# mduhme/fusion-gcn

Hardware: AMD Instinct MI355X
Metric: clips/sec (N,C,T,V,M)=(64,3,300,25,2) fwd+bwd (higher is better)
Workload: dtype f32 (products from exact 3-way bf16 splits; see notes.dtype); 1 GPU; AGCN 10-block fwd+bwd, NTU-RGB-D graph, synthetic (N,C,T,V,M)=(64,3,300,25,2), 60 classes, train-mode BatchNorm, CrossEntropy, all parameter gradients; global_batch=64, per_gpu_batch=64, parallelism=dp1, launch=hipgraph, input_pipeline=one HBM-resident batch, init_override=gcn1.bn.weight=1.0 (reference: 1e-6); see notes

## Files before the change

fusion_gcn_amd/csrc/fgcn_tconv.hip:

```cpp
#include "fgcn_tile.hpp"
#include <type_traits>

namespace fgcn {

struct HaloP {
    const float* in;
    float* out;
    const float* w4;
    const float* bias;
    float* stats;
    long long Mv;
    unsigned in_bytes, w_bytes, out_bytes;
    unsigned w_plane_bytes;
    int tiles_m, tiles_n, per_xcd;
    int Tv, V, K, N, ld_in, ld_out;
    FastDiv dV, dTvV, dTv;
    int T_in_full, in_s, in_o, Th_in;
    int T_out_full, out_s, out_o, Th_out;
    int taps, tb, tc;
    int dmin, halo_rows;
    int accumulate;
    const float* bn_a;
    const unsigned char* bn_mask;
    const float* bn_vec;
    const float* fin_vec;
    const float* fin_res;
    float* fin_out;
    unsigned char* fin_mask;
    const float* ep_vec;
    const float* ep_res;
    const float* ep_rvec;
    unsigned* in_amax;
    int stats_rows;
};

#ifndef FGCN_PROBE_HALO
#define FGCN_PROBE_HALO 0
#endif
#ifndef FGCN_HALO_RING
#define FGCN_HALO_RING 4
#endif
#ifndef FGCN_HALO_PF64
#define FGCN_HALO_PF64 1
#endif
constexpr int HAS = 36;
constexpr int HALO_MAX_STAGE = 13;
constexpr int XSB = 80;
using u32x4 = __attribute__((ext_vector_type(4))) unsigned int;

__device__ __forceinline__ f32x4 buf_load4(__amdgpu_buffer_rsrc_t r, unsigned voff, unsigned soff) {
    return __builtin_bit_cast(f32x4, __builtin_amdgcn_raw_buffer_load_b128(r, voff, soff, 0));
}

template <int NT, int MINB, int MM>
__global__ __launch_bounds__(256, MINB) void conv_halo_kernel(HaloP p) {
    extern __shared__ __attribute__((aligned(16))) float Ah[];
    const int tid = threadIdx.x, lane = tid & 63, wave = tid >> 6;
    const int l31 = lane & 31, h = lane >> 5;
    int bm, bn;
    if (p.per_xcd > 0) {
        const int vid = xcd_tile(blockIdx.x, p.per_xcd);
        if (vid >= p.tiles_m * p.tiles_n) return;
        bm = vid / p.tiles_n;
        bn = vid - bm * p.tiles_n;
    } else {
        bm = blockIdx.x;
        bn = blockIdx.y;
    }
    const long long m0 = (long long)bm * 128;
    const int n0 = bn * 32 * NT;
    const int V = p.V, TvV = p.Tv * p.V;
    const unsigned k4b = (tid & 7) * 16;

    const __amdgpu_buffer_rsrc_t rin = buffer_rsrc(p.in, p.in_bytes);
    const __amdgpu_buffer_rsrc_t rw = buffer_rsrc(p.w4, p.w_bytes);

    const long long mrow = m0 + wave * 32 + l31;
    const bool row_ok = mrow < p.Mv;
    const int th_lane = row_ok ? (int)(((unsigned)mrow / (unsigned)V) % (unsigned)p.Tv) : 0;

    unsigned src_off[HALO_MAX_STAGE];
    const int nstage = (p.halo_rows + 31) >> 5;
#pragma unroll
    for (int i = 0; i < HALO_MAX_STAGE; ++i) {
        src_off[i] = 0x80000000u;
        const int r = (tid >> 3) + 32 * i;
        const long long hv = m0 + (long long)p.dmin * V + r;
        if (i < nstage && hv >= 0 && hv < p.Mv) {
            const unsigned hu = (unsigned)hv;
            const int n = (int)(hu / (unsigned)TvV);
            const int rem = (int)(hu - (unsigned)n * (unsigned)TvV);
            const int th = (int)((unsigned)rem / (unsigned)V);
            const int v = rem - th * V;
            const int fr = th * p.in_s + p.in_o;
            if (th < p.Th_in && fr < p.T_in_full)
                src_off[i] = (unsigned)(((((long long)n * p.T_in_full + fr) * V + v) * p.ld_in) * 4) + k4b;
        }
    }

    f32x16 acc[NT];
#pragma unroll
    for (int i = 0; i < NT; ++i) acc[i] = zero16();

    const int IT = p.taps * 4;
    const int K4 = p.K >> 2;
    const int col = n0 + l31;
    unsigned wvoff[NT];
#pragma unroll
    for (int nt = 0; nt < NT; ++nt) wvoff[nt] = (unsigned)(((long long)h * p.N + col + nt * 32) * 16);
    const float* arow = &Ah[(wave * 32 + l31) * HAS + 4 * h];

    auto w_soff = [&](int it, int kc) -> unsigned {
        const int j = it >> 2, q = it & 3;
        return (unsigned)(((long long)(j * K4 + (kc >> 2) + 2 * q) * p.N) * 16);
    };
    auto a_read = [&](int it, bool& ok) -> f32x4 {
        const int j = it >> 2, q = it & 3;
        const int d = j * p.tb + p.tc;
        const int ts = th_lane + d;
        ok = row_ok && ts >= 0 && ts < p.Th_in;
        return *reinterpret_cast<const f32x4*>(arow + (d - p.dmin) * V * HAS + 8 * q);
    };

    for (int kc = 0; kc < p.K; kc += 32) {
        __syncthreads();
        {
            f32x4 stage[HALO_MAX_STAGE];
#pragma unroll
            for (int i = 0; i < HALO_MAX_STAGE; ++i)
                if (i < nstage) stage[i] = buf_load4(rin, src_off[i], (unsigned)kc * 4);
#pragma unroll
            for (int i = 0; i < HALO_MAX_STAGE; ++i) {
                const int r = (tid >> 3) + 32 * i;
                if (i < nstage && r < p.halo_rows) *reinterpret_cast<f32x4*>(&Ah[r * HAS + (tid & 7) * 4]) = stage[i];
            }
        }
        __syncthreads();

        f32x4 b0[NT], b1[NT];
        {
            const unsigned so = w_soff(0, kc);
#pragma unroll
            for (int nt = 0; nt < NT; ++nt) b0[nt] = buf_load4(rw, wvoff[nt], so);
        }
        bool ok0, ok1;
        f32x4 a0 = a_read(0, ok0), a1;
        for (int it = 0; it < IT; it += 2) {
            {
                const unsigned so = w_soff(it + 1, kc);
#pragma unroll
                for (int nt = 0; nt < NT; ++nt) b1[nt] = buf_load4(rw, wvoff[nt], so);
            }
            a1 = a_read(it + 1, ok1);
            if (!ok0) a0 = f32x4{0.f, 0.f, 0.f, 0.f};
            if constexpr (MM != 0) {
                const Frag<MM> ap = make_frag<MM>(a0);
#pragma unroll
                for (int nt = 0; nt < NT; ++nt) acc[nt] = mfma_frag<MM>(ap, make_frag<MM>(b0[nt]), acc[nt]);
            } else {
#pragma unroll
                for (int e = 0; e < 4; ++e)
#pragma unroll
                    for (int nt = 0; nt < NT; ++nt) acc[nt] = mfma32(a0[e], b0[nt][e], acc[nt]);
            }
            if (it + 2 < IT) {
                const unsigned so = w_soff(it + 2, kc);
#pragma unroll
                for (int nt = 0; nt < NT; ++nt) b0[nt] = buf_load4(rw, wvoff[nt], so);
                a0 = a_read(it + 2, ok0);
            }
            if (!ok1) a1 = f32x4{0.f, 0.f, 0.f, 0.f};
            if constexpr (MM != 0) {
                const Frag<MM> ap = make_frag<MM>(a1);
#pragma unroll
                for (int nt = 0; nt < NT; ++nt) acc[nt] = mfma_frag<MM>(ap, make_frag<MM>(b1[nt]), acc[nt]);
            } else {
#pragma unroll
                for (int e = 0; e < 4; ++e)
#pragma unroll
                    for (int nt = 0; nt < NT; ++nt) acc[nt] = mfma32(a1[e], b1[nt][e], acc[nt]);
            }
        }
    }


    const bool plain_out = p.out_s == 1 && p.out_o == 0 && p.T_out_full == p.Tv && p.Th_out == p.Tv;
    constexpr unsigned OOB = 0x80000000u;
    const __amdgpu_buffer_rsrc_t rout = buffer_rsrc(p.out, p.out_bytes);
    const __amdgpu_buffer_rsrc_t rbias = buffer_rsrc((p.bias ? p.bias : p.w4), p.bias ? (unsigned)p.N * 4u : 0u);
    float ssum[NT], ssq[NT], bv[NT];
#pragma unroll
    for (int nt = 0; nt < NT; ++nt) {
        ssum[nt] = 0.f;
        ssq[nt] = 0.f;
        bv[nt] = __builtin_bit_cast(float, __builtin_amdgcn_raw_buffer_load_b32(
                                               rbias, col + nt * 32 < p.N ? (unsigned)(col + nt * 32) * 4u : OOB, 0, 0));
    }
    unsigned rowoff[16];
#pragma unroll
    for (int r = 0; r < 16; ++r) {
        const long long m = m0 + wave * 32 + acc_row(r, lane);
        bool ok = m < p.Mv;
        unsigned orow = (unsigned)(ok ? m : 0);
        if (!plain_out) {
            const int n = (int)(orow / (unsigned)TvV);
            const int rem = (int)(orow - (unsigned)n * (unsigned)TvV);
            const int th = (int)((unsigned)rem / (unsigned)V);
            const int v = rem - th * V;
            ok = ok && th < p.Th_out;
            orow = (unsigned)((n * p.T_out_full + th * p.out_s + p.out_o) * V + v);
        }
        rowoff[r] = ok ? orow * (unsigned)p.ld_out * 4u : OOB;
    }
    auto epilogue = [&](auto acc_c) {
        constexpr bool ACC = decltype(acc_c)::value;
#pragma unroll
        for (int nt = 0; nt < NT; ++nt) {
            const int c = col + nt * 32;
            const unsigned coff = c < p.N ? (unsigned)c * 4u : OOB;
            float old[16];
#pragma unroll
            for (int r = 0; r < 16; ++r) {
                old[r] = 0.f;
                if constexpr (ACC)
                    old[r] = __builtin_bit_cast(float, __builtin_amdgcn_raw_buffer_load_b32(
                        rout, (rowoff[r] == OOB || coff == OOB) ? OOB : rowoff[r] + coff, 0, 0));
            }
#pragma unroll
            for (int r = 0; r < 16; ++r) {
                const unsigned off = (rowoff[r] == OOB || coff == OOB) ? OOB : rowoff[r] + coff;
                const float val = acc[nt][r] + bv[nt] + old[r];
                __builtin_amdgcn_raw_buffer_store_b32(__builtin_bit_cast(unsigned, val), rout, off, 0, 0);
                const float kept = off != OOB ? val : 0.f;
                ssum[nt] += kept;
                ssq[nt] += kept * kept;
            }
        }
    };
    if (p.accumulate) epilogue(std::true_type{});
    else epilogue(std::false_type{});
    if (p.stats) {
        constexpr int BN = 32 * NT;
        __syncthreads();
        float* red = Ah;
#pragma unroll
        for (int nt = 0; nt < NT; ++nt) {
            const float a = ssum[nt] + __shfl_xor(ssum[nt], 32);
            const float b = ssq[nt] + __shfl_xor(ssq[nt], 32);
            if (lane < 32) {
                red[(0 * 4 + wave) * BN + nt * 32 + lane] = a;
                red[(1 * 4 + wave) * BN + nt * 32 + lane] = b;
            }
        }
        __syncthreads();
        if (tid < 2 * BN) {
            const int which = tid / BN, c = tid - which * BN;
            if (n0 + c < p.N)
                p.stats[((long long)bm * 2 + which) * p.N + n0 + c] =
                    red[(which * 4 + 0) * BN + c] + red[(which * 4 + 1) * BN + c] + red[(which * 4 + 2) * BN + c] +
                    red[(which * 4 + 3) * BN + c];
        }
    }
}

template <int NT, int KC, int NP, int EPI = 0, bool FIN = false, int WR = 2, bool STR = false, int IN16 = 0>
__global__ __launch_bounds__(256, (NP == 1 && !FIN && EPI != 4) ? 3 : 2) void conv_halo_x3k32_kernel(HaloP p) {
    static_assert(!IN16 || (NP == 1 && !FIN), "bfloat16 input: the one-part kernel without the fused input stage");
    static_assert(IN16 != 2 || EPI == 0, "bfloat16 output: the plain store epilogue");
    constexpr bool O16 = IN16 == 2;
    static_assert(!(STR && EPI == 3), "an accumulating epilogue stores plainly");
    static_assert(WR == 2 || (WR == 4 && KC == 32 && !FIN), "wave arrangement: 2 x 2, or 4 x 1 for the tap form");
    static_assert(!FIN || KC == 32, "the fused input stage is built for the tap form (32-channel chunks)");
    static_assert((EPI == 0 || EPI == 2 || EPI == 3 || EPI == 4) && !(FIN && EPI != 0),
                  "epilogue: store / store + BatchNorm-backward sums / accumulate / inference output stage");
    constexpr int MTW = WR == 4 ? 3 : 4;
    constexpr int BMR = WR * 16 * MTW;
    static_assert(NP == 1 || NP == 2 || NP == 3, "one or three bf16 parts per operand, or two f16 parts (FGCN_PRODUCTS_F16X2)");
    static_assert(!(FIN && NP == 2), "the fused input stage is not built for the f16x2 products");
    static_assert((NT == 1 || NT == 2 || (NT == 4 && WR == 4)) && (KC == 32 || KC == 64), "wave tile is 64 rows x 32 or 64 columns (48 x 128 as 4 x 1 waves)");
    constexpr int XS = KC * 2;
    auto swz = [](int r) -> unsigned { return KC == 32 ? (unsigned)(r & 4) << 3 : (unsigned)(r & 6) << 4; };
    constexpr int TPR = KC / 4;
    constexpr int RPP = 256 / TPR;
    constexpr int SPC = KC / 32;
    constexpr bool PF = KC == 64 || (NT == 1 && NP == 3 && !FIN && FGCN_HALO_PF64);
    constexpr int NST = KC == 64 ? 8 : HALO_MAX_STAGE;
    constexpr int NU = 2 * NT;
#ifndef FGCN_HALO_RING_NP1
#define FGCN_HALO_RING_NP1 4
#endif
    constexpr int RS = (FGCN_HALO_RING == 4 && NU == 4 && (NP >= 2 || FGCN_HALO_RING_NP1 == 4) && (EPI != 2 || WR == 4) && !FIN) ? 4 : 2;
    constexpr unsigned OOB = 0x80000000u;
    extern __shared__ __attribute__((aligned(16))) float Ah[];
    const int tid = threadIdx.x, lane = tid & 63, wave = __builtin_amdgcn_readfirstlane(tid >> 6);
    const int l15 = lane & 15, g4 = lane >> 4;
    const int wr = WR == 4 ? wave : wave >> 1, wc = WR == 4 ? 0 : wave & 1;
    int bm = blockIdx.x, bn = blockIdx.y;
    if (p.per_xcd > 0) {
        const int vid = xcd_tile(blockIdx.x, p.per_xcd);
        if (vid >= p.tiles_m * p.tiles_n) return;
        bm = vid / p.tiles_n;
        bn = vid - bm * p.tiles_n;
    }
    const int m0 = bm * BMR;
    const int Mv = (int)p.Mv;
    constexpr int BN = (4 / WR) * NT * 32;
    const int n0 = bn * BN;
    const int V = p.V, TvV = p.Tv * p.V;
    const unsigned k4b = (tid % TPR) * 16;

    const __amdgpu_buffer_rsrc_t rin = buffer_rsrc(p.in, p.in_bytes);
    const __amdgpu_buffer_rsrc_t rw = buffer_rsrc((reinterpret_cast<const unsigned char*>(p.w4) + (NP == 2 ? 16 : 0)), p.w_bytes);
    constexpr int EA_NONE = 1000;
    const int ew = NP == 2 ? min(scale_exp_for(*reinterpret_cast<const unsigned*>(p.w4)), 126) : 0;
    int ea = EA_NONE, abound = 0;

    bool row_ok[MTW];
    int th_lane[MTW];
#pragma unroll
    for (int mt = 0; mt < MTW; ++mt) {
        const int mrow = m0 + wr * (16 * MTW) + mt * 16 + l15;
        row_ok[mt] = mrow < Mv;
        const unsigned fr_all = fastdiv(row_ok[mt] ? (unsigned)mrow : 0u, p.dV);
        th_lane[mt] = (int)(fr_all - fastdiv(fr_all, p.dTv) * (unsigned)p.Tv);
    }

    unsigned src_off[NST];
    const int nstage = (p.halo_rows + RPP - 1) / RPP;
#pragma unroll
    for (int i = 0; i < NST; ++i) {
        src_off[i] = OOB;
        const int r = tid / TPR + RPP * i;
        const int hv = m0 + p.dmin * V + r;
        if (i < nstage && hv >= 0 && hv < Mv) {
            const unsigned hu = (unsigned)hv;
            const int n = (int)fastdiv(hu, p.dTvV);
            const int rem = (int)(hu - (unsigned)n * (unsigned)TvV);
            const int th = (int)fastdiv((unsigned)rem, p.dV);
            const int v = rem - th * V;
            const int fr = th * p.in_s + p.in_o;
            if (th < p.Th_in && fr < p.T_in_full)
                src_off[i] = (unsigned)(((n * p.T_in_full + fr) * V + v) * p.ld_in) * 4u + k4b;
        }
    }

    f32x4 acc[MTW][NU];
#pragma unroll
    for (int mt = 0; mt < MTW; ++mt)
#pragma unroll
        for (int nu = 0; nu < NU; ++nu) acc[mt][nu] = f32x4{0.f, 0.f, 0.f, 0.f};

    const int col = n0 + wc * NT * 32 + l15;
    unsigned wvoff[NU];
#pragma unroll
    for (int nu = 0; nu < NU; ++nu) wvoff[nu] = (unsigned)(((long long)g4 * p.N + col + nu * 16) * 16);

    unsigned char* Xh = reinterpret_cast<unsigned char*>(Ah);
    const unsigned plane = (unsigned)p.halo_rows * XS;
    const int xrow = wr * (16 * MTW) + l15;
    const int IT2 = p.taps * SPC;
    const int K8 = p.K >> 3;
    bool probe_started = false;
    auto load_w = [&](u32x4v (&dst)[NP], int nu, int it, int kc) {
        if (it >= IT2) {
            it -= IT2;
            kc += KC;
        }
        if (kc >= p.K) {
            it = 0;
            kc = 0;
        }
        const int j = it / SPC, s2 = it - j * SPC;
        const unsigned so = (unsigned)(((long long)(j * K8 + (kc >> 3) + 4 * s2) * p.N) * 16);
        if ((FGCN_PROBE_HALO & 16) && probe_started) return;
#pragma unroll
        for (int pl = 0; pl < NP; ++pl)
            dst[pl] = __builtin_amdgcn_raw_buffer_load_b128(rw, wvoff[nu], so + pl * p.w_plane_bytes, 0);
    };
    auto load_a = [&](u32x4v (&dst)[NP], int mt, int it) {
        if ((FGCN_PROBE_HALO & 8) && it > 0) return;
        const int j = it / SPC, s2 = it - j * SPC;
        const int d = j * p.tb + p.tc;
        const int r = xrow + (d - p.dmin) * V + mt * 16;
        const unsigned char* src = Xh + r * XS + ((unsigned)(16 * g4 + 64 * s2) ^ swz(r));
        const int ts = th_lane[mt] + d;
        const bool ok = row_ok[mt] && ts >= 0 && ts < p.Th_in;
#pragma unroll
        for (int pl = 0; pl < NP; ++pl) {
            const u32x4v v = *reinterpret_cast<const u32x4v*>(src + pl * plane);
            dst[pl] = ok ? v : u32x4v{0u, 0u, 0u, 0u};
        }
    };

    f32x4 stage[NST], stage2[FIN ? NST : 1];
    constexpr int HALF = FIN ? (NST + 1) / 2 : NST;
    auto fetch = [&](int kc, int lo = 0, int hi = 64) {
#pragma unroll
        for (int i = 0; i < NST; ++i)
            if (i >= lo && i < hi && i < nstage) {
                if constexpr (IN16) {
                    const u32x2 h2 = __builtin_bit_cast(u32x2, __builtin_amdgcn_raw_buffer_load_b64(rin, src_off[i] == OOB ? OOB : src_off[i] >> 1, (unsigned)kc * 2, 0));
                    const unsigned b0 = h2[0], b1 = h2[1];
                    stage[i] = f32x4{__builtin_bit_cast(float, b0), __builtin_bit_cast(float, b1), 0.f, 0.f};
                    continue;
                }
                stage[i] = buf_load4(rin, src_off[i], (unsigned)kc * 4);
                if constexpr (FIN)
                    stage2[i] = buf_load4(buffer_rsrc(p.fin_res, p.in_bytes), src_off[i],
                                          (unsigned)kc * 4);
            }
    };
    auto deposit = [&](int kc, int lo = 0, int hi = 64) {
        const float a_scale = (NP == 2 && ea != EA_NONE) ? exp2i(ea) : 1.f;
        f32x4 fsc = {0.f, 0.f, 0.f, 0.f}, fsh = fsc;
        const __amdgpu_buffer_rsrc_t rgo = buffer_rsrc((FIN ? (void*)p.fin_out : (void*)p.out), FIN ? p.in_bytes : 0u);
        const __amdgpu_buffer_rsrc_t rgm = buffer_rsrc((FIN ? (void*)p.fin_mask : (void*)p.out), FIN ? p.in_bytes >> 5 : 0u);
        const int own0 = -p.dmin * V;
        if constexpr (FIN) {
            fsc = *reinterpret_cast<const f32x4*>(p.fin_vec + 2 * p.K + kc + (tid % TPR) * 4);
            fsh = *reinterpret_cast<const f32x4*>(p.fin_vec + 3 * p.K + kc + (tid % TPR) * 4);
        }
#pragma unroll
        for (int i = 0; i < NST; ++i) {
            if (i < lo || i >= hi) continue;
            const int r = tid / TPR + RPP * i;
            if constexpr (FIN) {
                if (i < nstage) {
                    const bool live = src_off[i] != OOB;
                    f32x4 v = stage[i] * fsc + fsh + stage2[i];
#pragma unroll
                    for (int e = 0; e < 4; ++e) v[e] = live ? fmaxf(v[e], 0.f) : 0.f;
                    stage[i] = v;
                    const bool mine = live && bn == 0 && r >= own0 && r < own0 + BMR;
                    __builtin_amdgcn_raw_buffer_store_b128(__builtin_bit_cast(u32x4, v), rgo, mine ? src_off[i] : OOB,
                                                           (unsigned)kc * 4, 0);
                    unsigned w = ((v[0] > 0.f ? 1u : 0u) | (v[1] > 0.f ? 2u : 0u) | (v[2] > 0.f ? 4u : 0u) | (v[3] > 0.f ? 8u : 0u))
                                 << (4 * (lane & 7));
                    w |= (unsigned)__shfl_xor((int)w, 1);
                    w |= (unsigned)__shfl_xor((int)w, 2);
                    w |= (unsigned)__shfl_xor((int)w, 4);
                    __builtin_amdgcn_raw_buffer_store_b32(w, rgm, (mine && (lane & 7) == 0) ? (src_off[i] + (unsigned)kc * 4) >> 5 : OOB,
                                                          0, 0);
                }
            }
            if (i < nstage && r < p.halo_rows) {
                u32x2 ph, pm, pl;
                unsigned char* dst = Xh + r * XS + ((unsigned)((tid % TPR) * 8) ^ swz(r));
                if constexpr (NP == 2) {
                    split2h_x4(stage[i] * a_scale, ph, pm);
                    *reinterpret_cast<u32x2*>(dst) = ph;
                    *reinterpret_cast<u32x2*>(dst + plane) = pm;
                    continue;
                }
                if constexpr (IN16) {
                    const float e0 = stage[i][0], e1 = stage[i][1];
                    *reinterpret_cast<u32x2*>(dst) = u32x2{__builtin_bit_cast(unsigned, e0), __builtin_bit_cast(unsigned, e1)};
                    continue;
                }
                split3_x4(stage[i], ph, pm, pl);
                *reinterpret_cast<u32x2*>(dst) = ph;
                if constexpr (NP == 3) {
                    *reinterpret_cast<u32x2*>(dst + plane) = pm;
                    *reinterpret_cast<u32x2*>(dst + 2 * plane) = pl;
                }
            }
        }
    };

    u32x4v a[MTW][NP], wq[RS][NP];
#pragma unroll
    for (int nu = 0; nu < RS - 1; ++nu) load_w(wq[nu], nu, 0, 0);
    if constexpr (PF) fetch(0);
    float* smax = reinterpret_cast<float*>(Xh + NP * plane);
    auto chunk_max = [&]() {
        float m = 0.f;
#pragma unroll
        for (int i = 0; i < NST; ++i)
            if (i < nstage)
                m = fmaxf(fmaxf(m, fmaxf(fabsf(stage[i][0]), fabsf(stage[i][1]))), fmaxf(fabsf(stage[i][2]), fabsf(stage[i][3])));
#pragma unroll
        for (int d = 32; d >= 1; d >>= 1) m = fmaxf(m, __shfl_xor(m, d));
        if (lane == 0) smax[wave] = m;
    };
    for (int kc = 0; kc < p.K; kc += KC) {
        if constexpr (NP == 2 && PF) chunk_max();
        __syncthreads();
        if constexpr (FIN) {
            fetch(kc, 0, HALF);
            deposit(kc, 0, HALF);
            fetch(kc, HALF, NST);
            deposit(kc, HALF, NST);
        } else if ((FGCN_PROBE_HALO & 4) && probe_started) {
        } else {
            if constexpr (!PF) fetch(kc);
            if constexpr (NP == 2) {
                if constexpr (!PF) {
                    chunk_max();
                    __syncthreads();
                }
                const unsigned mb = __builtin_bit_cast(unsigned, fmaxf(fmaxf(smax[0], smax[1]), fmaxf(smax[2], smax[3])));
                const int ec = __builtin_amdgcn_readfirstlane((mb >> 23) == 0u ? EA_NONE : min(scale_exp_for(mb), 126));
                if (p.in_amax && tid == 0 && bn == 0) atomicMax(p.in_amax, mb);
                if (ec != EA_NONE && ec != ea) {
                    int d = ea == EA_NONE ? 0 : ec - ea;
                    if (d > 120 - abound) d = 120 - abound;
                    if (ea == EA_NONE) ea = ec;
                    else if (d != 0) {
                        const float f = exp2i(d);
#pragma unroll
                        for (int mt = 0; mt < MTW; ++mt)
#pragma unroll
                            for (int nu = 0; nu < NU; ++nu) acc[mt][nu] *= f;
                        ea += d;
                        abound += d;
                    }
                }
                abound = (abound > 44 ? abound : 44) + 1;
            }
            deposit(kc);
        }
        __syncthreads();
        if constexpr (PF) {
            if (kc + KC < p.K) fetch(kc + KC);
        }
#pragma unroll
        for (int mt = 0; mt < MTW; ++mt) load_a(a[mt], mt, 0);
#pragma unroll 1
        for (int it = 0; it < IT2; ++it) {
            const int itn = it + 1 < IT2 ? it + 1 : it;
#pragma unroll
            for (int nu = 0; nu < NU; ++nu) {
                const int t = nu + RS - 1;
                if (t < NU) load_w(wq[t % RS], t, it, kc);
                else load_w(wq[t % RS], t - NU, it + 1, kc);
#pragma unroll
                for (int mt = 0; mt < MTW; ++mt) {
                    if constexpr ((FGCN_PROBE_HALO & 2) != 0) acc[mt][nu][0] += __builtin_bit_cast(float, a[mt][0][0] ^ wq[nu % RS][0][0] ^ a[mt][NP - 1][3] ^ wq[nu % RS][NP - 1][3]);
                    else if constexpr (NP == 3) acc[mt][nu] = mfma_x3_k32(a[mt], wq[nu % RS], acc[mt][nu]);
                    else if constexpr (NP == 2) acc[mt][nu] = mfma_h2_k32(a[mt], wq[nu % RS], acc[mt][nu]);
                    else acc[mt][nu] = mfma_bf16_k32(a[mt][0], wq[nu % RS][0], acc[mt][nu]);
                    if (nu == NU - 1) load_a(a[mt], mt, itn);
                }
            }
        }
        probe_started = true;
    }

    __builtin_amdgcn_sched_barrier(0);
    const bool plain_out = p.out_s == 1 && p.out_o == 0 && p.T_out_full == p.Tv && p.Th_out == p.Tv;
    const __amdgpu_buffer_rsrc_t rout = buffer_rsrc(p.out, p.out_bytes);
    const __amdgpu_buffer_rsrc_t rbias = buffer_rsrc((p.bias ? p.bias : p.w4), p.bias ? (unsigned)p.N * 4u : 0u);
    float ssum[NU], ssq[NU], bv[NU];
    unsigned coff[NU];
    const float un_a = (NP == 2 && ea != EA_NONE) ? exp2i(-ea) : 1.f, un_w = NP == 2 ? exp2i(-ew) : 1.f;
    constexpr bool bnb = EPI == 2;
    const __amdgpu_buffer_rsrc_t rba = buffer_rsrc((bnb ? p.bn_a : p.out), p.out_bytes);
    const __amdgpu_buffer_rsrc_t rbm = buffer_rsrc((bnb ? (const void*)p.bn_mask : (const void*)p.out), p.out_bytes >> 5);
    const __amdgpu_buffer_rsrc_t rbv = buffer_rsrc((bnb ? p.bn_vec : p.w4), bnb ? (unsigned)p.N * 8u : 0u);
    float bmean[NU], brstd[NU];
#pragma unroll
    for (int nu = 0; nu < NU; ++nu) {
        ssum[nu] = 0.f;
        ssq[nu] = 0.f;
        coff[nu] = col + nu * 16 < p.N ? (unsigned)(col + nu * 16) * 4u : OOB;
        bv[nu] = __builtin_bit_cast(float, __builtin_amdgcn_raw_buffer_load_b32(rbias, coff[nu], 0, 0));
        bmean[nu] = bnb ? __builtin_bit_cast(float, __builtin_amdgcn_raw_buffer_load_b32(rbv, coff[nu], 0, 0)) : 0.f;
        brstd[nu] = bnb ? __builtin_bit_cast(float, __builtin_amdgcn_raw_buffer_load_b32(rbv, coff[nu], (unsigned)p.N * 4u, 0)) : 0.f;
    }
    unsigned rowoff[MTW][4];
#pragma unroll
    for (int mt = 0; mt < MTW; ++mt)
#pragma unroll
        for (int r = 0; r < 4; ++r) {
            const int m = m0 + wr * (16 * MTW) + mt * 16 + 4 * g4 + r;
            bool ok = m < Mv;
            unsigned orow = (unsigned)(ok ? m : 0);
            if (!plain_out) {
                const int n = (int)fastdiv(orow, p.dTvV);
                const int rem = (int)(orow - (unsigned)n * (unsigned)TvV);
                const int th = (int)fastdiv((unsigned)rem, p.dV);
                const int v = rem - th * V;
                ok = ok && th < p.Th_out;
                orow = (unsigned)((n * p.T_out_full + th * p.out_s + p.out_o) * V + v);
            }
            rowoff[mt][r] = ok ? orow * (unsigned)p.ld_out * 4u : OOB;
        }
    float av[bnb ? 2 : 1][NU][4];
    unsigned mbits[bnb ? 2 : 1][NU][4];
    auto load_bn = [&](int mt, float (&a_)[NU][4], unsigned (&m_)[NU][4]) {
#pragma unroll
        for (int nu = 0; nu < NU; ++nu)
#pragma unroll
            for (int r = 0; r < 4; ++r) {
                const unsigned off = (rowoff[mt][r] == OOB || coff[nu] == OOB) ? OOB : rowoff[mt][r] + coff[nu];
                a_[nu][r] = __builtin_bit_cast(float, __builtin_amdgcn_raw_buffer_load_b32(rba, off, 0, 0));
                m_[nu][r] = (unsigned)__builtin_amdgcn_raw_buffer_load_b8(rbm, off == OOB ? OOB : off >> 5, 0, 0);
            }
    };
    constexpr bool fep = EPI == 4;
    constexpr bool ldacc = EPI == 3 || fep;
    const __amdgpu_buffer_rsrc_t rold = fep ? buffer_rsrc((p.ep_res ? (const void*)p.ep_res : (const void*)p.out), p.ep_res ? p.out_bytes : 0u)
                                            : rout;
    float esc[NU], esh[NU], rsc[NU], rsh[NU];
    if constexpr (fep) {
        const __amdgpu_buffer_rsrc_t rv = buffer_rsrc(p.ep_vec, (unsigned)p.N * 16u);
        const __amdgpu_buffer_rsrc_t rrv = buffer_rsrc((p.ep_rvec ? p.ep_rvec : p.ep_vec), p.ep_rvec ? (unsigned)p.N * 16u : 0u);
        const float res_unit = p.ep_rvec ? 0.f : 1.f;
#pragma unroll
        for (int nu = 0; nu < NU; ++nu) {
            esc[nu] = __builtin_bit_cast(float, __builtin_amdgcn_raw_buffer_load_b32(rv, coff[nu], (unsigned)p.N * 8u, 0));
            esh[nu] = __builtin_fmaf(bv[nu], esc[nu], __builtin_bit_cast(float, __builtin_amdgcn_raw_buffer_load_b32(rv, coff[nu], (unsigned)p.N * 12u, 0)));
            rsc[nu] = __builtin_bit_cast(float, __builtin_amdgcn_raw_buffer_load_b32(rrv, coff[nu], (unsigned)p.N * 8u, 0)) + res_unit;
            rsh[nu] = __builtin_bit_cast(float, __builtin_amdgcn_raw_buffer_load_b32(rrv, coff[nu], (unsigned)p.N * 12u, 0));
        }
    }
    float oldv[ldacc ? 2 : 1][NU][4];
    auto load_old = [&](int mt, float (&o_)[NU][4]) {
#pragma unroll
        for (int nu = 0; nu < NU; ++nu)
#pragma unroll
            for (int r = 0; r < 4; ++r)
                o_[nu][r] = __builtin_bit_cast(float, __builtin_amdgcn_raw_buffer_load_b32(
                    rold, (rowoff[mt][r] == OOB || coff[nu] == OOB) ? OOB : rowoff[mt][r] + coff[nu], 0, 0));
    };
    if constexpr (bnb) load_bn(0, av[0], mbits[0]);
    if constexpr (ldacc) load_old(0, oldv[0]);
#pragma unroll
    for (int mt = 0; mt < MTW; ++mt) {
        if constexpr (bnb) {
            if (mt + 1 < MTW) load_bn(mt + 1, av[(mt + 1) & 1], mbits[(mt + 1) & 1]);
        }
        if constexpr (ldacc) {
            if (mt + 1 < MTW) load_old(mt + 1, oldv[(mt + 1) & 1]);
        }
        if constexpr (O16) {
            const bool odd = lane & 1;
#pragma unroll
            for (int rp = 0; rp < 4; rp += 2) {
#pragma unroll
                for (int nu = 0; nu < NU; ++nu) {
                    const unsigned off0 = (rowoff[mt][rp] == OOB || coff[nu] == OOB) ? OOB : rowoff[mt][rp] + coff[nu];
                    const unsigned off1 = (rowoff[mt][rp + 1] == OOB || coff[nu] == OOB) ? OOB : rowoff[mt][rp + 1] + coff[nu];
                    const float v0 = acc[mt][nu][rp] + bv[nu], v1 = acc[mt][nu][rp + 1] + bv[nu];
                    const float other = lane_xor1(odd ? v0 : v1);
                    const unsigned pk = odd ? pack_bf16x2(other, v1) : pack_bf16x2(v0, other);
                    const unsigned mine = odd ? off1 : off0;
                    __builtin_amdgcn_raw_buffer_store_b32(pk, rout, mine == OOB ? OOB : (mine - (odd ? 4u : 0u)) >> 1, 0, STR ? FGCN_STORE_AUX : 0);
                    const float k0 = off0 != OOB ? v0 : 0.f, k1 = off1 != OOB ? v1 : 0.f;
                    ssum[nu] += k0;
                    ssq[nu] = __builtin_fmaf(k0, k0, ssq[nu]);
                    ssum[nu] += k1;
                    ssq[nu] = __builtin_fmaf(k1, k1, ssq[nu]);
                }
            }
            continue;
        }
#pragma unroll
        for (int r = 0; r < 4; ++r) {
#pragma unroll
            for (int nu = 0; nu < NU; ++nu) {
                const unsigned off = (rowoff[mt][r] == OOB || coff[nu] == OOB) ? OOB : rowoff[mt][r] + coff[nu];
                float val = (NP == 2 ? acc[mt][nu][r] * un_a * un_w : acc[mt][nu][r]) + bv[nu];
                if constexpr (fep) {
                    val = __builtin_fmaf(acc[mt][nu][r], esc[nu], esh[nu]) + __builtin_fmaf(oldv[mt & 1][nu][r], rsc[nu], rsh[nu]);
                    val = fmaxf(val, 0.f);
                } else if constexpr (ldacc) {
                    val += oldv[mt & 1][nu][r];
                }
                __builtin_amdgcn_raw_buffer_store_b32(__builtin_bit_cast(unsigned, val), rout, ((FGCN_PROBE_HALO & 1) && val != 123.456f) ? OOB : off, 0, STR ? FGCN_STORE_AUX : 0);
                const float kept = off != OOB ? val : 0.f;
                if constexpr (bnb) {
                    const float dp = (mbits[mt & 1][nu][r] >> ((off >> 2) & 7u)) & 1u ? kept : 0.f;
                    ssum[nu] += dp;
                    ssq[nu] = __builtin_fmaf(dp, (av[mt & 1][nu][r] - bmean[nu]) * brstd[nu], ssq[nu]);
                } else {
                    ssum[nu] += kept;
                    ssq[nu] = __builtin_fmaf(kept, kept, ssq[nu]);
                }
            }
        }
        if constexpr (bnb || ldacc) __builtin_amdgcn_sched_barrier(0);
    }
    if (p.stats && !((FGCN_PROBE_HALO & 32) && ssum[0] != 123.456f)) {
        __syncthreads();
        float* red = Ah;
#pragma unroll
        for (int nu = 0; nu < NU; ++nu) {
            float sa = ssum[nu] + __shfl_xor(ssum[nu], 16);
            float sb = ssq[nu] + __shfl_xor(ssq[nu], 16);
            sa += __shfl_xor(sa, 32);
            sb += __shfl_xor(sb, 32);
            if (lane < 16) {
                red[(0 * WR + wr) * BN + wc * NT * 32 + nu * 16 + lane] = sa;
                red[(1 * WR + wr) * BN + wc * NT * 32 + nu * 16 + lane] = sb;
            }
        }
        __syncthreads();
        if (tid < 2 * BN) {
            const int which = tid / BN, c = tid - which * BN;
            if (n0 + c < p.N) {
                float t = red[(which * WR + 0) * BN + c] + red[(which * WR + 1) * BN + c];
                if constexpr (WR == 4) t = (t + red[(which * WR + 2) * BN + c]) + red[(which * WR + 3) * BN + c];
                p.stats[((long long)bm * 2 + which) * p.N + n0 + c] = t;
                if constexpr (WR == 4) {
                    const long long extra = (long long)bm + p.tiles_m;
                    if (extra < p.stats_rows) p.stats[(extra * 2 + which) * p.N + n0 + c] = 0.f;
                }
            }
        }
    }
}

}

using namespace fgcn;

static int halo_tile_rows(int V) {
    const bool k32 = fgcn::math_mode() == FGCN_MATH_BF16 || fgcn::math_mode() == FGCN_MATH_BF16X3;
    return (k32 && (128 + 8 * V) * 64 * 3 > 80 * 1024) ? 96 : 128;
}

extern "C" int fgcn_tconv_halo_bn_sums(void) {
    const int mm = fgcn::math_mode();
    return (mm == FGCN_MATH_BF16 || mm == FGCN_MATH_BF16X3) ? 1 : 0;
}

extern "C" int fgcn_tconv_halo_tiles(int B, int Th_out, int Th_in, int V) {
    const int Tv = Th_out > Th_in ? Th_out : Th_in;
    return (int)cdiv((long long)B * Tv * V, halo_tile_rows(V));
}

constexpr bool halo_k32_built(int NT, int KC, int NP, int EPI, bool FIN, int WR, bool STR, int H16) {
    if ((STR && EPI == 3) || (EPI == 4 && NP == 2)) return false;
    if (H16 && !(NP == 1 && !FIN && KC == 32 && EPI != 4 && (H16 == 1 || EPI == 0))) return false;
    if (FIN) return NT <= 2 && KC == 32 && NP != 2 && EPI == 0 && WR == 2;
    if (KC == 64) return NT <= 2 && WR == 2 && (EPI == 0 || EPI == 3);
    if (WR == 2) return NT <= 2;
    return NT == 2 || (NT == 4 && (EPI == 0 || EPI == 3));
}

static int tconv_halo_impl(const float* in, float* out, const float* w4, const float* bias, float* stat_partials,
                           int B, int Th, int V, int K, int N, int ld_in, int ld_out,
                           int T_in_full, int in_s, int in_o, int Th_in,
                           int T_out_full, int out_s, int out_o,
                           int taps, int tb, int tc, int accumulate, const float* bn_a, const unsigned char* bn_mask,
                           const float* bn_vec, const float* fin_vec, const float* fin_res, float* fin_out,
                           unsigned char* fin_mask, unsigned* in_amax, void* stream, int half_mask, const float* ep_vec,
                           const float* ep_res, const float* ep_rvec) {
    const bool in16 = half_mask & 1, out16 = half_mask & 2;
    FGCN_REQUIRE(in && out && w4, FGCN_E_BADARG, "tconv_halo: null pointer");
    const bool fep = ep_vec != nullptr;
    FGCN_REQUIRE(!fep || ((fgcn::math_mode() == FGCN_MATH_BF16X3 || fgcn::math_mode() == FGCN_MATH_BF16) && !fgcn::f16x2_products() && !in16 &&
                          !accumulate && !bn_a && !stat_partials && !(fin_vec || fin_res || fin_out || fin_mask) && taps > 1 && out_s == 1 && out_o == 0 &&
                          T_out_full == Th && aligned16(ep_vec) && (!ep_res || aligned16(ep_res)) && (!ep_rvec || ep_res)),
                 FGCN_E_BADARG, "tconv_halo_bn_relu: the inference output stage needs the split kernel (bf16x3 products or bf16), the tap form, a "
                 "plain output view, no statistics / accumulation / fused input stage");
    FGCN_REQUIRE(!in16 || (fgcn::math_mode() == FGCN_MATH_BF16 && !(fin_vec || fin_res || fin_out || fin_mask) && !(taps == 1 && K % 64 == 0)),
                 FGCN_E_BADARG, "tconv_halo: a bfloat16 input needs math mode bf16, the tap form and no fused input stage");
    FGCN_REQUIRE(!out16 || (!accumulate && !bn_a && !fep && ld_out % 2 == 0), FGCN_E_BADARG,
                 "tconv_halo: a bfloat16 output is written by the plain store epilogue (no accumulation, no BatchNorm-backward sums)");
    const bool fin = fin_vec || fin_res || fin_out || fin_mask;
    FGCN_REQUIRE(!fin || !fgcn::f16x2_products(), FGCN_E_BADARG, "tconv_halo: the fused input stage is not built for the f16x2 products");
    FGCN_REQUIRE(!fin || (fin_vec && fin_res && fin_out && fin_mask && fgcn_tconv_halo_bn_sums() && !bn_a && !accumulate && taps > 1 &&
                          ld_in == K && in_s == 1 && in_o == 0 && Th_in == T_in_full && Th_in == Th && aligned16(fin_res) &&
                          aligned16(fin_out) && aligned16(fin_vec) && ((uintptr_t)fin_mask & 3u) == 0),
                 FGCN_E_BADARG, "tconv_halo: the fused input stage (BatchNorm + shortcut + ReLU while the image is staged) needs the "
                 "split-bf16 kernel, all four of (vec, shortcut, G, sign image), a plain contiguous input view (ld_in == K) and taps > 1");
    FGCN_REQUIRE(!bn_a || (bn_mask && bn_vec && stat_partials && fgcn_tconv_halo_bn_sums() && ld_out == N && N % 8 == 0 &&
                           out_s == 1 && out_o == 0 && T_out_full == Th),
                 FGCN_E_BADARG, "tconv_halo: BatchNorm-backward sums need the split-bf16 kernel, a contiguous plain output (ld_out == N, "
                 "N %% 8 == 0), the sign image, the coefficient vector and a partials buffer");
    FGCN_REQUIRE(B > 0 && Th > 0 && V > 0 && V <= FGCN_MAX_V && K > 0 && N > 0, FGCN_E_BADARG,
                 "tconv_halo: bad sizes B=%d Th=%d V=%d K=%d N=%d", B, Th, V, K, N);
    FGCN_REQUIRE(K % 32 == 0 && N % 4 == 0 && ld_in % 4 == 0 && ld_out % 4 == 0 && ld_in >= K && ld_out >= N, FGCN_E_ALIGN,
                 "tconv_halo: K must be a multiple of 32, N and strides multiples of 4 (K=%d N=%d ld_in=%d ld_out=%d)", K,
                 N, ld_in, ld_out);
    FGCN_REQUIRE(aligned16(in) && aligned16(w4), FGCN_E_ALIGN, "tconv_halo: 16-byte alignment");
    FGCN_REQUIRE(taps >= 1 && taps <= 16 && (tb == 1 || tb == -1), FGCN_E_BADARG, "tconv_halo: taps=%d tb=%d", taps, tb);
    FGCN_REQUIRE(in_s >= 1 && out_s >= 1 && in_o >= 0 && out_o >= 0 && Th_in > 0, FGCN_E_BADARG,
                 "tconv_halo: bad frame views");
    FGCN_REQUIRE((long long)(Th_in - 1) * in_s + in_o < T_in_full && (long long)(Th - 1) * out_s + out_o < T_out_full,
                 FGCN_E_BADARG, "tconv_halo: frame view exceeds the tensor (Th=%d Th_in=%d)", Th, Th_in);
    const int mm = fgcn::math_mode();
    const long long in_bytes = (long long)B * T_in_full * V * ld_in * (in16 ? 2 : 4);
    const bool two = fgcn::f16x2_products();
    const long long w_bytes = (long long)taps * K * N * (mm != FGCN_MATH_F32 ? (two ? 4 : 6) : 4);
    const long long out_bytes = (long long)B * T_out_full * V * ld_out * (out16 ? 2 : 4);
    FGCN_REQUIRE(fits_buffer(in_bytes) && fits_buffer(w_bytes) && fits_buffer(out_bytes), FGCN_E_BADARG,
                 "tconv_halo: tensors must be smaller than 2 GiB (32-bit buffer offsets)");
    HaloP p;
    p.in = in; p.out = out; p.w4 = w4; p.bias = bias; p.stats = stat_partials;
    p.in_bytes = (unsigned)in_bytes; p.w_bytes = (unsigned)w_bytes; p.out_bytes = (unsigned)out_bytes;
    p.w_plane_bytes = (unsigned)((long long)taps * K * N * 2);
    p.Tv = Th > Th_in ? Th : Th_in;
    p.Mv = (long long)B * p.Tv * V;
    p.V = V; p.K = K; p.N = N; p.ld_in = ld_in; p.ld_out = ld_out;
    p.dV = make_fastdiv((unsigned)V); p.dTvV = make_fastdiv((unsigned)(p.Tv * V)); p.dTv = make_fastdiv((unsigned)p.Tv);
    FGCN_REQUIRE(mm == FGCN_MATH_F32 || p.Mv < (1ll << 29), FGCN_E_BADARG, "tconv_halo: too many rows for the split kernels' index arithmetic (< 2^29)");
    p.T_in_full = T_in_full; p.in_s = in_s; p.in_o = in_o; p.Th_in = Th_in;
    p.T_out_full = T_out_full; p.out_s = out_s; p.out_o = out_o; p.Th_out = Th;
    p.taps = taps; p.tb = tb; p.tc = tc; p.accumulate = accumulate;
    p.bn_a = bn_a; p.bn_mask = bn_mask; p.bn_vec = bn_vec;
    p.fin_vec = fin_vec; p.fin_res = fin_res; p.fin_out = fin_out; p.fin_mask = fin_mask;
    p.ep_vec = ep_vec; p.ep_res = ep_res; p.ep_rvec = ep_rvec;
    p.in_amax = fgcn::f16x2_products() ? in_amax : nullptr;
    const int d0 = tc, d1 = (taps - 1) * tb + tc;
    p.dmin = d0 < d1 ? d0 : d1;
    const int dmax = d0 < d1 ? d1 : d0;
    int bmr = halo_tile_rows(V);
    p.stats_rows = (int)cdiv(p.Mv, bmr);
    const bool wide128 = ((fgcn::tuning(7) & 16) || (N <= 128 && !(fgcn::tuning(7) & 32) && mm != FGCN_MATH_BF16)) && N > 64 && !bn_a && !fep;
    const bool wide_rows = (mm == FGCN_MATH_BF16X3 || (mm == FGCN_MATH_BF16 && (fgcn::tuning(7) & 16))) && ((N <= 64 && N > 32) || wide128) && !(taps == 1 && K % 64 == 0) &&
                           !(fin_vec || fin_res || fin_out || fin_mask) && !(fgcn::tuning(7) & 8) &&
                           192 + (dmax - p.dmin) * V <= 32 * HALO_MAX_STAGE && (size_t)(192 + (dmax - p.dmin) * V) * 64 * 3 + 16 <= 80 * 1024 &&
                           (cdiv(p.Mv, 192) >= 1536 || (fgcn::tuning(7) & 64));
    if (wide_rows) bmr = 192;
    p.halo_rows = bmr + (dmax - p.dmin) * V;
    FGCN_REQUIRE(p.halo_rows <= 32 * HALO_MAX_STAGE, FGCN_E_BADARG, "tconv_halo: halo of %d rows too large", p.halo_rows);
    const size_t lds = mm == FGCN_MATH_BF16X3 ? (size_t)p.halo_rows * XSB * 3 : (size_t)p.halo_rows * HAS * sizeof(float);
    const long long tiles = cdiv(p.Mv, bmr);
    FGCN_REQUIRE(p.Mv < (1ll << 31) - 4096, FGCN_E_BADARG, "tconv_halo: too many rows (32-bit row indices)");
    hipStream_t s = (hipStream_t)stream;
    constexpr int max_lds = 32 * HALO_MAX_STAGE * XSB * 3;
    const bool three = fgcn::tuning(4) == 0;
    p.tiles_m = (int)tiles;
    p.tiles_n = (int)cdiv(N, N <= 64 ? 64 : 128);
    dim3 grid((unsigned)tiles, (unsigned)p.tiles_n);
    p.per_xcd = 0;
    if (mm == FGCN_MATH_BF16X3 || mm == FGCN_MATH_BF16) {
        const bool one = mm == FGCN_MATH_BF16;
        const bool pw = taps == 1 && K % 64 == 0;
        if (!(fgcn::tuning(5) & 32) && tiles * p.tiles_n < (1ll << 30)) {
            p.per_xcd = (int)cdiv(tiles * p.tiles_n, 8);
            grid = dim3((unsigned)(p.per_xcd * 8));
        }
        const int np = one ? 1 : (two ? 2 : 3);
        const size_t lds_k = (pw ? (size_t)bmr * 128 * np : (size_t)p.halo_rows * 64 * np) + 16;
        FGCN_REQUIRE(bmr == 128 || wide_rows, FGCN_E_BADARG, "tconv_halo: the split kernels run the 128-row tile (V <= %d)", FGCN_MAX_V);
        FGCN_REQUIRE(!(bn_a && accumulate), FGCN_E_BADARG, "tconv_halo: BatchNorm-backward sums of an accumulating call are not built");
        const int epi = fep ? 4 : (bn_a ? 2 : (accumulate ? 3 : 0));
        const bool stream_k = !out16 ? fgcn::stream_out((long long)B * Th * V * N * 4) : ((fgcn::tuning(25) & 1) && fgcn::stream_out((long long)B * Th * V * N * 2));
        FGCN_REQUIRE(!fin || !pw, FGCN_E_BADARG, "tconv_halo: the fused input stage runs on the 128-row tap tile (V <= 32)");
        FGCN_REQUIRE(!pw || epi == 0 || epi == 3, FGCN_E_BADARG, "tconv_halo: BatchNorm-backward sums are built for the tap kernel only");
        const int nt = !wide_rows ? (N <= 64 ? 1 : 2) : (epi != 4 && N > 64 ? 4 : 2);
        const int h16 = !(one && !fin && !pw && epi != 4) ? 0 : (out16 && epi == 0 ? 2 : (in16 ? 1 : 0));
        const int kc = pw ? 64 : 32, wr = wide_rows ? 4 : 2;
        const bool str = epi != 3 && stream_k;
        const bool built = dispatch(
            [&](auto NT, auto KC, auto NP, auto EPI, auto FIN, auto WR, auto STR, auto H16) {
                constexpr bool built = halo_k32_built(NT, KC, NP, EPI, FIN == 1, WR, STR == 1, H16);
                if constexpr (built) launch_lds<conv_halo_x3k32_kernel<NT, KC, NP, EPI, FIN == 1, WR, STR == 1, H16>>(grid, dim3(256), max_lds, lds_k, s, p);
                return built;
            },
            one_of<1, 2, 4>{nt}, one_of<32, 64>{kc}, one_of<1, 2, 3>{np}, one_of<0, 2, 3, 4>{epi}, one_of<0, 1>{fin}, one_of<2, 4>{wr},
            one_of<0, 1>{str}, one_of<0, 1, 2>{h16});
        FGCN_REQUIRE(built, FGCN_E_BADARG, "tconv_halo: no such kernel form");
        return launch_status("tconv_halo");
    }
    if ((fgcn::tuning(5) & 2) && tiles * p.tiles_n < (1ll << 30)) {
        p.per_xcd = (int)cdiv(tiles * p.tiles_n, 8);
        grid = dim3((unsigned)(p.per_xcd * 8));
    }
    const bool built = dispatch(
        [&](auto NT, auto MB, auto BF) {
            launch_lds<conv_halo_kernel<NT, MB, BF>>(grid, dim3(256), max_lds, lds, s, p);
            return true;
        },
        one_of<2, 4>{N <= 64 ? 2 : 4}, one_of<2, 3>{three ? 3 : 2}, one_of<0, 1>{mm == FGCN_MATH_BF16});
    FGCN_REQUIRE(built, FGCN_E_BADARG, "tconv_halo: no such kernel form");
    return launch_status("tconv_halo");
}

extern "C" int fgcn_tconv_halo(const void* in, void* out, const float* w4, const float* bias, float* stat_partials,
                               int B, int Th, int V, int K, int N, int ld_in, int ld_out,
                               int T_in_full, int in_s, int in_o, int Th_in,
                               int T_out_full, int out_s, int out_o,
                               int taps, int tb, int tc, int accumulate, const float* bn_a, const unsigned char* bn_mask,
                               const float* bn_vec, const float* fin_vec, const float* fin_res, float* fin_out,
                               unsigned char* fin_mask, unsigned* in_amax, int half_mask, void* stream) {
    FGCN_REQUIRE(half_mask == 0 || half_mask == 1 || half_mask == 3, FGCN_E_BADARG, "tconv_halo: half_mask=%d (0, 1 or 3)", half_mask);
    return tconv_halo_impl(static_cast<const float*>(in), static_cast<float*>(out), w4, bias, stat_partials, B, Th, V, K, N, ld_in, ld_out, T_in_full,
                           in_s, in_o, Th_in, T_out_full, out_s, out_o, taps, tb, tc, accumulate, bn_a, bn_mask, bn_vec, fin_vec, fin_res, fin_out,
                           fin_mask, in_amax, stream, half_mask, nullptr, nullptr, nullptr);
}

extern "C" int fgcn_tconv_halo_bn_relu(const float* in, float* out, const float* w4, const float* bias, const float* bn_vec,
                                       const float* res, const float* res_vec, int B, int T, int V, int K, int N, int ld_in, int ld_out,
                                       int taps, int tb, int tc, void* stream) {
    FGCN_REQUIRE(bn_vec, FGCN_E_BADARG, "tconv_halo_bn_relu: the BatchNorm vector is required");
    return tconv_halo_impl(in, out, w4, bias, nullptr, B, T, V, K, N, ld_in, ld_out, T, 1, 0, T, T, 1, 0, taps, tb, tc, 0, nullptr, nullptr, nullptr,
                           nullptr, nullptr, nullptr, nullptr, nullptr, stream, 0, bn_vec, res, res_vec);
}
```

Before: 1187 clips/s.

## Tile temporal conv rows over joint groups to shrink the halo

Reinterprets the temporal conv rows so each tile covers a subset of joints (G groups of g joints, default the largest divisor of V up to 5) instead of all V joints per frame. The halo then spans (dmax-dmin)*g rows instead of (dmax-dmin)*V, cutting redundant halo loads and LDS per tile. When the halo fits, a shorter staging-array variant is launched. The cost is extra index arithmetic (a division by G) in both the load and store address paths, loss of the plain-output fast path, and more tiles per batch.

```diff
diff --git a/fusion_gcn_amd/csrc/fgcn_tconv.hip b/fusion_gcn_amd/csrc/fgcn_tconv.hip
--- a/fusion_gcn_amd/csrc/fgcn_tconv.hip
+++ b/fusion_gcn_amd/csrc/fgcn_tconv.hip
@@ -15,6 +15,8 @@
     int tiles_m, tiles_n, per_xcd;
     int Tv, V, K, N, ld_in, ld_out;
     FastDiv dV, dTvV, dTv;
+    int Vf, G;
+    FastDiv dG;
     int T_in_full, in_s, in_o, Th_in;
     int T_out_full, out_s, out_o, Th_out;
     int taps, tb, tc;
@@ -45,6 +47,7 @@
 #endif
 constexpr int HAS = 36;
 constexpr int HALO_MAX_STAGE = 13;
+constexpr int HALO_GROUP_STAGE = 8;
 constexpr int XSB = 80;
 using u32x4 = __attribute__((ext_vector_type(4))) unsigned int;
 
@@ -263,9 +266,11 @@
     }
 }
 
-template <int NT, int KC, int NP, int EPI = 0, bool FIN = false, int WR = 2, bool STR = false, int IN16 = 0>
+template <int NT, int KC, int NP, int EPI = 0, bool FIN = false, int WR = 2, bool STR = false, int IN16 = 0, int JG = 0>
 __global__ __launch_bounds__(256, (NP == 1 && !FIN && EPI != 4) ? 3 : 2) void conv_halo_x3k32_kernel(HaloP p) {
     static_assert(!IN16 || (NP == 1 && !FIN), "bfloat16 input: the one-part kernel without the fused input stage");
+    static_assert(!JG || KC == 32, "joint groups: the tap form");
+    static_assert(JG != 2 || (WR == 4 && NT == 2 && NP == 3 && !FIN), "rows requested a chunk ahead: the 4 x 1 form over 64 columns");
     static_assert(IN16 != 2 || EPI == 0, "bfloat16 output: the plain store epilogue");
     constexpr bool O16 = IN16 == 2;
     static_assert(!(STR && EPI == 3), "an accumulating epilogue stores plainly");
@@ -283,8 +288,8 @@
     constexpr int TPR = KC / 4;
     constexpr int RPP = 256 / TPR;
     constexpr int SPC = KC / 32;
-    constexpr bool PF = KC == 64 || (NT == 1 && NP == 3 && !FIN && FGCN_HALO_PF64);
-    constexpr int NST = KC == 64 ? 8 : HALO_MAX_STAGE;
+    constexpr bool PF = KC == 64 || (NT == 1 && NP == 3 && !FIN && FGCN_HALO_PF64) || JG == 2;
+    constexpr int NST = (KC == 64 || JG) ? HALO_GROUP_STAGE : HALO_MAX_STAGE;
     constexpr int NU = 2 * NT;
 #ifndef FGCN_HALO_RING_NP1
 #define FGCN_HALO_RING_NP1 4
@@ -337,10 +342,15 @@
             const int n = (int)fastdiv(hu, p.dTvV);
             const int rem = (int)(hu - (unsigned)n * (unsigned)TvV);
             const int th = (int)fastdiv((unsigned)rem, p.dV);
-            const int v = rem - th * V;
+            int v = rem - th * V;
             const int fr = th * p.in_s + p.in_o;
+            int ns = n;
+            if (p.G > 1) {
+                ns = (int)fastdiv((unsigned)n, p.dG);
+                v += (n - ns * p.G) * V;
+            }
             if (th < p.Th_in && fr < p.T_in_full)
-                src_off[i] = (unsigned)(((n * p.T_in_full + fr) * V + v) * p.ld_in) * 4u + k4b;
+                src_off[i] = (unsigned)(((ns * p.T_in_full + fr) * p.Vf + v) * p.ld_in) * 4u + k4b;
         }
     }
 
@@ -547,7 +557,7 @@
     }
 
     __builtin_amdgcn_sched_barrier(0);
-    const bool plain_out = p.out_s == 1 && p.out_o == 0 && p.T_out_full == p.Tv && p.Th_out == p.Tv;
+    const bool plain_out = p.out_s == 1 && p.out_o == 0 && p.T_out_full == p.Tv && p.Th_out == p.Tv && p.G == 1;
     const __amdgpu_buffer_rsrc_t rout = buffer_rsrc(p.out, p.out_bytes);
     const __amdgpu_buffer_rsrc_t rbias = buffer_rsrc((p.bias ? p.bias : p.w4), p.bias ? (unsigned)p.N * 4u : 0u);
     float ssum[NU], ssq[NU], bv[NU];
@@ -579,9 +589,10 @@
                 const int n = (int)fastdiv(orow, p.dTvV);
                 const int rem = (int)(orow - (unsigned)n * (unsigned)TvV);
                 const int th = (int)fastdiv((unsigned)rem, p.dV);
-                const int v = rem - th * V;
+                const int ns = (int)fastdiv((unsigned)n, p.dG);
+                const int v = rem - th * V + (n - ns * p.G) * V;
                 ok = ok && th < p.Th_out;
-                orow = (unsigned)((n * p.T_out_full + th * p.out_s + p.out_o) * V + v);
+                orow = (unsigned)((ns * p.T_out_full + th * p.out_s + p.out_o) * p.Vf + v);
             }
             rowoff[mt][r] = ok ? orow * (unsigned)p.ld_out * 4u : OOB;
         }
@@ -720,6 +731,17 @@
     return (k32 && (128 + 8 * V) * 64 * 3 > 80 * 1024) ? 96 : 128;
 }
 
+static int halo_joint_group(int V, int N, int np) {
+    const int key = fgcn::tuning(27);
+    if (key == 1) return V;
+    if (key == -1) return 1;
+    if (key >= 2) return key;
+    (void)N; (void)np;
+    for (int g = V < 5 ? V : 5; g > 1; --g)
+        if (V % g == 0) return g;
+    return 1;
+}
+
 extern "C" int fgcn_tconv_halo_bn_sums(void) {
     const int mm = fgcn::math_mode();
     return (mm == FGCN_MATH_BF16 || mm == FGCN_MATH_BF16X3) ? 1 : 0;
@@ -730,7 +752,9 @@
     return (int)cdiv((long long)B * Tv * V, halo_tile_rows(V));
 }
 
-constexpr bool halo_k32_built(int NT, int KC, int NP, int EPI, bool FIN, int WR, bool STR, int H16) {
+constexpr bool halo_k32_built(int NT, int KC, int NP, int EPI, bool FIN, int WR, bool STR, int H16, int JG) {
+    if (JG && KC != 32) return false;
+    if (JG == 2 && !(WR == 4 && NT == 2 && NP == 3 && !FIN && EPI != 4)) return false;
     if ((STR && EPI == 3) || (EPI == 4 && NP == 2)) return false;
     if (H16 && !(NP == 1 && !FIN && KC == 32 && EPI != 4 && (H16 == 1 || EPI == 0))) return false;
     if (FIN) return NT <= 2 && KC == 32 && NP != 2 && EPI == 0 && WR == 2;
@@ -794,8 +818,15 @@
     p.w_plane_bytes = (unsigned)((long long)taps * K * N * 2);
     p.Tv = Th > Th_in ? Th : Th_in;
     p.Mv = (long long)B * p.Tv * V;
-    p.V = V; p.K = K; p.N = N; p.ld_in = ld_in; p.ld_out = ld_out;
-    p.dV = make_fastdiv((unsigned)V); p.dTvV = make_fastdiv((unsigned)(p.Tv * V)); p.dTv = make_fastdiv((unsigned)p.Tv);
+    p.K = K; p.N = N; p.ld_in = ld_in; p.ld_out = ld_out;
+    const int key_g = fgcn::tuning(27);
+    FGCN_REQUIRE(key_g >= -1 && (key_g <= 1 || (key_g <= V && V % key_g == 0)), FGCN_E_BADARG,
+                 "tconv_halo: tuning key 27 = %d joints per group does not divide V = %d", key_g, V);
+    const bool grouped = (mm == FGCN_MATH_BF16X3 || mm == FGCN_MATH_BF16) && taps > 1;
+    const int g = !grouped ? V : halo_joint_group(V, N, mm == FGCN_MATH_BF16 ? 1 : (two ? 2 : 3));
+    p.V = g; p.Vf = V; p.G = V / g;
+    p.dV = make_fastdiv((unsigned)g); p.dTvV = make_fastdiv((unsigned)(p.Tv * g)); p.dTv = make_fastdiv((unsigned)p.Tv);
+    p.dG = make_fastdiv((unsigned)p.G);
     FGCN_REQUIRE(mm == FGCN_MATH_F32 || p.Mv < (1ll << 29), FGCN_E_BADARG, "tconv_halo: too many rows for the split kernels' index arithmetic (< 2^29)");
     p.T_in_full = T_in_full; p.in_s = in_s; p.in_o = in_o; p.Th_in = Th_in;
     p.T_out_full = T_out_full; p.out_s = out_s; p.out_o = out_o; p.Th_out = Th;
@@ -812,10 +843,10 @@
     const bool wide128 = ((fgcn::tuning(7) & 16) || (N <= 128 && !(fgcn::tuning(7) & 32) && mm != FGCN_MATH_BF16)) && N > 64 && !bn_a && !fep;
     const bool wide_rows = (mm == FGCN_MATH_BF16X3 || (mm == FGCN_MATH_BF16 && (fgcn::tuning(7) & 16))) && ((N <= 64 && N > 32) || wide128) && !(taps == 1 && K % 64 == 0) &&
                            !(fin_vec || fin_res || fin_out || fin_mask) && !(fgcn::tuning(7) & 8) &&
-                           192 + (dmax - p.dmin) * V <= 32 * HALO_MAX_STAGE && (size_t)(192 + (dmax - p.dmin) * V) * 64 * 3 + 16 <= 80 * 1024 &&
+                           192 + (dmax - p.dmin) * g <= 32 * HALO_MAX_STAGE && (size_t)(192 + (dmax - p.dmin) * g) * 64 * 3 + 16 <= 80 * 1024 &&
                            (cdiv(p.Mv, 192) >= 1536 || (fgcn::tuning(7) & 64));
     if (wide_rows) bmr = 192;
-    p.halo_rows = bmr + (dmax - p.dmin) * V;
+    p.halo_rows = bmr + (dmax - p.dmin) * g;
     FGCN_REQUIRE(p.halo_rows <= 32 * HALO_MAX_STAGE, FGCN_E_BADARG, "tconv_halo: halo of %d rows too large", p.halo_rows);
     const size_t lds = mm == FGCN_MATH_BF16X3 ? (size_t)p.halo_rows * XSB * 3 : (size_t)p.halo_rows * HAS * sizeof(float);
     const long long tiles = cdiv(p.Mv, bmr);
@@ -846,14 +877,16 @@
         const int h16 = !(one && !fin && !pw && epi != 4) ? 0 : (out16 && epi == 0 ? 2 : (in16 ? 1 : 0));
         const int kc = pw ? 64 : 32, wr = wide_rows ? 4 : 2;
         const bool str = epi != 3 && stream_k;
+        const bool short_stage = p.G > 1 && !pw && p.halo_rows <= 32 * HALO_GROUP_STAGE && !(fgcn::tuning(7) & 256);
+        const int jg = !short_stage ? 0 : ((wr == 4 && nt == 2 && np == 3 && !fin && epi != 4 && (fgcn::tuning(7) & 128)) ? 2 : 1);
         const bool built = dispatch(
-            [&](auto NT, auto KC, auto NP, auto EPI, auto FIN, auto WR, auto STR, auto H16) {
-                constexpr bool built = halo_k32_built(NT, KC, NP, EPI, FIN == 1, WR, STR == 1, H16);
-                if constexpr (built) launch_lds<conv_halo_x3k32_kernel<NT, KC, NP, EPI, FIN == 1, WR, STR == 1, H16>>(grid, dim3(256), max_lds, lds_k, s, p);
+            [&](auto NT, auto KC, auto NP, auto EPI, auto FIN, auto WR, auto STR, auto H16, auto JG) {
+                constexpr bool built = halo_k32_built(NT, KC, NP, EPI, FIN == 1, WR, STR == 1, H16, JG);
+                if constexpr (built) launch_lds<conv_halo_x3k32_kernel<NT, KC, NP, EPI, FIN == 1, WR, STR == 1, H16, JG>>(grid, dim3(256), max_lds, lds_k, s, p);
                 return built;
             },
             one_of<1, 2, 4>{nt}, one_of<32, 64>{kc}, one_of<1, 2, 3>{np}, one_of<0, 2, 3, 4>{epi}, one_of<0, 1>{fin}, one_of<2, 4>{wr},
-            one_of<0, 1>{str}, one_of<0, 1, 2>{h16});
+            one_of<0, 1>{str}, one_of<0, 1, 2>{h16}, one_of<0, 1, 2>{jg});
         FGCN_REQUIRE(built, FGCN_E_BADARG, "tconv_halo: no such kernel form");
         return launch_status("tconv_halo");
     }
```

New measurement: 1193 clips/s (median of 6 runs). Within noise of the previous version (+0.5%).
